# Litianyu141/Pytorch-Sparse-Linalg-torch-amgx.cg.bicg.gmres

Measured on AMD Instinct MI355X. Metric: cg_iters_per_sec, higher is better.
Workload: dtype f64

## Files before the change

pytorch-sparse-linalg-torch-amgx.cg.bicg.gmres_amd/csrc/hipk_cg.hip:

```cpp
#include <type_traits>
#include <math.h>
#include <stdlib.h>

#include <vector>

#include "hipk_blas1.h"
#include "hipk_solve.h"
#include "hipk_spmv.h"
#include "hipk_handoff.h"
#include "hipk_fx.h"

struct hipk_lds_ctl {
    double rs_last;
    int64_t it_done;
    int32_t redo;
    int32_t bar;
    unsigned xcc_mask;
    unsigned pad;
};
struct hipk_cg_scal {
    double gamma[2];
    double atol2;
    double bs;
    double res2;
// ... 949 lines not shown
    }
    if (wg == 0 && tid == 0) {
        a.gamma[it & 1] = gamma;
        scal->rs_last = rs_last;
        scal->it_done = it;
        if (done && it < stop0) *a.stop_it = it;
    }
}

__global__ __launch_bounds__(HIPK_THREADS) void hipk_cg_final_kernel(hipk_cg_scal *__restrict__ scal, int g,
                                                                     const double *__restrict__ part_res,
                                                                     const double *__restrict__ part_xx) {
    __shared__ double sbuf[2 * HIPK_THREADS];
    double res2, xx;
    hipk_reduce_parts2(part_res, part_xx, g, res2, xx, sbuf);
    if (threadIdx.x == 0) {
        scal->res2 = res2;
        scal->xx = xx;
    }
}


static constexpr int kCg2MaxChunks = 150;

static inline bool hipk_cg_streams_by_size(size_t n, size_t sv) { return 4 * n * sv > (size_t)384 << 20; }

#define HIPK_MID_ROW(W, NCH, PRE)                                                                                          \
    {W, NCH, PRE, hipk_cg_mid_kernel<T, W, NCH, PRE>,                                                                      \
     HIPK_FORM_OF_T(T, "hipk_cg_mid_kernel<", #W "," #NCH "," #PRE ">")}
template <typename T>
static const hipk_mid_entry<hipk_cg_mid_args> hipk_cg_mid_table[] = {
    HIPK_MID_ROW(5, 1, false), HIPK_MID_ROW(7, 1, false), HIPK_MID_ROW(9, 1, false), HIPK_MID_ROW(12, 1, false),
    HIPK_MID_ROW(5, 2, false), HIPK_MID_ROW(7, 2, false),
    HIPK_MID_ROW(5, 1, true),  HIPK_MID_ROW(7, 1, true),  HIPK_MID_ROW(9, 1, true),  HIPK_MID_ROW(12, 1, true)};
#undef HIPK_MID_ROW
static constexpr int kPcgMidMaxChunks = 256;
static constexpr size_t kPcgMidSlotBytes = 3 * (size_t)kMidMaxChunks * 256;

struct hipk_cg_layout {
    size_t scal;
    size_t part_a, part_b, part_c;
    size_t part_z[2];
    size_t part_d;
    size_t r, p, Ap;
    size_t lds_flags;
    size_t lds_rr_sub;
    size_t lds_rz_sub;
    bool mid;
    size_t ll_bytes;
    size_t r_ll;
    size_t pap_ll, rr_ll, rz_ll;
    bool fourth_vector;
    size_t p2;
    size_t fuse_words, fuse_ctl;
    size_t total;
};
static constexpr size_t kFuseBytes = 2 * (kFuseWordsBytes + kFuseCtlBytes);
static_assert(kFuseWordsBytes % 256 == 0 && kFuseCtlBytes == 8 * 16 * kFuseReplicaSlots, "the replicas follow the words, 128 bytes apart");
static_assert(kFuseBytes == 2 * (kFuseWordsBytes + kFuseCtlBytes) && (kFuseWordsBytes + kFuseCtlBytes) % 256 == 0,
              "the direction tail's words and replicas follow the first pair, laid out the same");
static_assert(kFuseBytes <= (size_t)kMidMaxChunks * HIPK_BASE_CHUNK * sizeof(double),
              "the fused form runs beyond the mid loop's chunk count, fp64: Ap is longer than its region");
static constexpr size_t kMidSlotArray = (size_t)kMidMaxChunks * 256;
static_assert(kMidSlotBytes == 2 * kMidSlotArray && kPcgMidSlotBytes == 3 * kMidSlotArray, "pap_ll, rr_ll and (pcg) rz_ll");
static_assert(HIPK_MAX_PARTS / 2 + 2 * kHoMaxWg <= HIPK_MAX_PARTS, "the LDS loop's hand-off flags fit the upper half of the spare slot");
static_assert(kHoMaxWg <= HIPK_MAX_PARTS, "the LDS loop's sub-partials fit a chunk-partial slot");
static_assert(kMidSlotBytes >= 256, "p2 ends inside the mid loop's bytes: 2 vec <= ll_bytes + 256");
static_assert(HIPK_SCRATCH_SLOTS == 4, "cg: part_a, part_b, part_c and one unused slot");

static hipk_cg_layout hipk_cg_make_layout(int64_t n, int dtype, bool pre) {
    const size_t sv = (dtype == HIPK_F64) ? 8 : 4, rows = (size_t)(n > 0 ? n : 1), vec = hipk_align_up(rows * sv, 256);
    const size_t slot = HIPK_MAX_PARTS * sizeof(double);
    const hipk_geom gm = hipk_make_geom(n > 0 ? n : 1);
    hipk_cg_layout L;
    hipk_carve take;
    L.scal = take(256);
    L.part_a = take(slot);
    L.part_b = take(slot);
    L.part_c = take(slot);
    L.part_z[0] = take(slot);
    L.part_z[1] = pre ? take(slot) : 0;
    L.part_d = pre ? take(slot) : L.part_a;
    L.lds_flags = L.part_c + slot / 2;
    L.lds_rr_sub = L.part_b;
    L.lds_rz_sub = L.part_z[1];
    L.r = take(vec);
    L.p = take(vec);
    L.mid = gm.g > kMidMinChunks && gm.g <= (pre ? kPcgMidMaxChunks : kMidMaxChunks);
    L.ll_bytes = hipk_align_up(rows * 16, 256);
    L.Ap = L.r_ll = take(L.mid ? L.ll_bytes : vec);
    L.pap_ll = L.mid ? take(pre ? kPcgMidSlotBytes : kMidSlotBytes) : 0;
    L.rr_ll = L.pap_ll + kMidSlotArray;
    L.rz_ll = L.rr_ll + kMidSlotArray;
    const bool second_p = !pre && !L.mid && gm.g > kMidMaxChunks && !hipk_cg_streams_by_size(rows, sv);
    L.p2 = L.Ap + vec;
    if (second_p) take(vec);
    L.fourth_vector = !pre && (L.mid || second_p);
    L.fuse_words = L.Ap;
    L.fuse_ctl = L.Ap + kFuseWordsBytes;
    L.total = take.o;
    return L;
}
extern "C" size_t hipk_cg_work_bytes(int64_t n, int dtype) { return hipk_cg_make_layout(n, dtype, false).total; }
extern "C" size_t hipk_pcg_work_bytes(int64_t n, int dtype) { return hipk_cg_make_layout(n, dtype, true).total; }

struct hipk_cg_path {
    bool small = false;
    bool streams = false;
    bool flat_dir = false;
    bool mid = false;
    const hipk_mid_entry<hipk_cg_mid_args> *mid_entry = nullptr;
    hipk_mid_plan mid_plan;
    size_t mid_lds = 0;
    int nch = 1, slot_stride = 16, xcd_aware = 1;
    bool lds_loop = false;
    bool spread = false;
    bool local = false;
    int64_t max_its = 0;
    bool two_launch = false;
    bool defer_x = false;
    bool fuse_update = false;
    bool fuse_dir = false;
    bool fuse_keep_p = false;
    void (*fuse_kern)(hipk_spmv_args, hipk_cg_fuse_args) = nullptr;
    hipk_spmv_args fuse_sa;
};

template <typename T, bool PRE>
static hipk_cg_path hipk_cg_path_begin(hipk_csr_s *A, const hipk_params *prm, int64_t maxiter, bool mid_failed, hipStream_t stream) {
    const int64_t n = A->n_rows;
    const int g = A->geom.g;
    hipk_cg_path path;
    if (!PRE) {
        path.small = g <= 8 && !hipk_sw_present("HIPK_CG_NO_SMALL");
        path.streams = hipk_sw_force("HIPK_CG_STREAMS", hipk_cg_streams_by_size((size_t)n, sizeof(T)));
        path.flat_dir = hipk_sw_force("HIPK_CG_FLAT_DIRECTION", (size_t)n * sizeof(T) > ((size_t)256 << 20));
    }
    path.nch = (PRE || g <= A->n_cu) ? 1 : 2;
    const int nch = path.nch;
    path.mid_entry = hipk_mid_pick(hipk_cg_mid_table<T>, A->max_row_len, nch, PRE);
    auto mid_lds = [nch](int slots) { return hipk_cg_mid_lds_bytes(slots * HIPK_TILE, nch, PRE, sizeof(T)); };
    path.mid = g > kMidMinChunks && g <= (PRE ? kPcgMidMaxChunks : kMidMaxChunks) && (!PRE || g <= A->n_cu) && A->geom.ch == HIPK_BASE_CHUNK &&
               A->op_cb == nullptr && A->crow != nullptr && A->max_row_len <= 12 && prm->profile == 0 && maxiter > 0 && !mid_failed &&
               hipk_sw_enabled("HIPK_CG_MID") && !hipk_sw_present("HIPK_CG_NO_LDS_LOOP") && !hipk_sw_present("HIPK_CG_NO_SMALL") &&
               path.mid_entry && hipk_mid_eligible(A, path.mid_entry, (g + nch - 1) / nch, mid_lds, stream, &path.mid_plan, &path.mid_lds);
    if (path.mid) {
        const int stride = g <= 32 ? 1 : g <= 256 ? 16 : 4;
        path.slot_stride = PRE ? stride : (int)hipk_sw_int("HIPK_CG_MID_STRIDE", stride);
        if (path.slot_stride < 1 || path.slot_stride > 16) path.slot_stride = 16;
        path.xcd_aware = PRE || hipk_sw_enabled("HIPK_CG_MID_XCD");
        path.max_its = hipk_sw_int("HIPK_CG_LAUNCH_ITS", 16384, 1);
    }
// ... 641 lines not shown
        const int grid1 = ((ntiles + 7) >> 3) << 3;
        for (; it <= maxiter; ++it) {
            HIPK_CHECK_HIP(pace.gate(it, stream, &stop));
            if (stop <= it) break;
            ca.it = it;
            ca.p_old = pbuf[it & 1];
            ca.p_new = pbuf[(it + 1) & 1];
            hipk_cg2_spmv_kernel<T, kCap2><<<grid1, HIPK_THREADS, 0, stream>>>(ca);
            if (it < maxiter)
                hipk_cg2_update_kernel<T><<<gm.g, HIPK_THREADS, 0, stream>>>(n, gm.ch, gm.g, scal, it, A->tile_part, ntiles, Ap,
                                                                            (const T *)pbuf[(it + 1) & 1], r, x, part_b);
            if ((it & 63) == 63) HIPK_CHECK_HIP(hipGetLastError());
        }
        if (it > maxiter) it = maxiter;
        return HIPK_OK;
    }

    int deferred_x_sequence() {
        T *pbuf[2] = {p_first ? hipk_at<T>(work, lay.p2) : p, p_first ? p : hipk_at<T>(work, lay.p2)};
        const int64_t it0 = it;
        if (path.fuse_update) HIPK_TRY(fuse_begin());
        for (; it < maxiter; ++it) {
            HIPK_CHECK_HIP(pace.gate(it, stream, &stop));
            if (stop <= it) break;
            const int j = (int)((it - it0) & 1);
            if (path.fuse_dir) {
                fuse_launch(it0, pbuf[j], pbuf[j ^ 1], j ? x : nullptr);
                if ((it & 63) == 63) HIPK_CHECK_HIP(hipGetLastError());
                continue;
            }
            if (path.fuse_update) {
                fuse_launch(it0, pbuf[j]);
            } else {
                sa.it = it;
                sa.x = sa.w = pbuf[j];
                HIPK_TRY(hipk_launch_spmv(A, sa, stream, &prof));
                hipk_cg_update_kernel<T><<<gm.g, HIPK_THREADS, 0, stream>>>(n, gm.ch, gm.g, scal, it, part_a, Ap, r, part_b, 0, &scal->alpha[it & 1]);
            }
            if (j == 0)
                hipk_cg_pdir_kernel<T><<<gm.g, HIPK_THREADS, 0, stream>>>(n, gm.ch, gm.g, scal, it, maxiter, part_b, r, pbuf[0], pbuf[1]);
            else
                hipk_cg_xdir_kernel<T><<<gm.g, HIPK_THREADS, 0, stream>>>(n, gm.ch, gm.g, scal, it, maxiter, part_b, r, pbuf[1], pbuf[0], x);
            if ((it & 63) == 63) HIPK_CHECK_HIP(hipGetLastError());
        }
        hipk_cg_xflush_kernel<T><<<gm.g, HIPK_THREADS, 0, stream>>>(n, gm.ch, scal, it, it0, pbuf[0], x, path.fuse_dir ? 1 : 0);
        return path.fuse_update ? fuse_end(it0, true, pbuf) : HIPK_OK;
    }

    int fuse_begin() {
        HIPK_CHECK_HIP(hipMemsetAsync(hipk_at<char>(work, lay.fuse_words), 0, kFuseBytes, stream));
        HIPK_CHECK_HIP(hipMemsetAsync(&scal->ctl, 0, sizeof(hipk_lds_ctl), stream));
        fuse_give_up_at = hipk_sw_present("HIPK_TEST_CG_FUSE_GIVE_UP") ? hipk_sw_int("HIPK_TEST_CG_FUSE_GIVE_UP", -1) : -1;
        fuse_dir_give_up_at = hipk_sw_present("HIPK_TEST_CG_FUSE_DIR_GIVE_UP") ? hipk_sw_int("HIPK_TEST_CG_FUSE_DIR_GIVE_UP", -1) : -1;
        fuse_note();
        return HIPK_OK;
    }
    void fuse_note() const {
        char name[64];
        snprintf(name, sizeof(name), "hipk_cg_fuse_update_kernel<%d>", A->sell_w);
        hipk_note_spmv_kernel(name);
    }
    void fuse_launch(int64_t it0, const T *pk, T *p_next = nullptr, T *xq = nullptr) {
        hipk_spmv_args fa = path.fuse_sa;
        fa.it = it;
        fa.x = fa.w = pk;
        hipk_cg_fuse_args ff;
        ff.scal = (hipk_cg_scal *)scal;
        ff.r = (double *)r;
        ff.part_rr = part_b;
        ff.part_pap = part_a;
        ff.words = hipk_at<char>(work, lay.fuse_words);
        ff.ctl = hipk_at<char>(work, lay.fuse_ctl);
        ff.seq = (unsigned)(it - it0) + 1u;
        ff.give_up = it == fuse_give_up_at ? 1 : 0;
        ff.p_next = (double *)p_next;
        ff.x = (double *)xq;
        ff.maxiter = maxiter;
        ff.keep_p = p_next != nullptr && path.fuse_keep_p ? 1 : 0;
        ff.dir_give_up = p_next != nullptr && it == fuse_dir_give_up_at ? 1 : 0;
        path.fuse_kern<<<hipk_xcd_grid(gm.g), HIPK_THREADS, 0, stream>>>(fa, ff);
    }
    int fuse_end(int64_t it0, bool deferred, T *const *pbuf = nullptr) {
        S hs;
        HIPK_CHECK_HIP(hipGetLastError());
        HIPK_CHECK_HIP(hipMemcpyAsync(&hs, scal, sizeof(hs), hipMemcpyDeviceToHost, stream));
        HIPK_CHECK_HIP(hipStreamSynchronize(stream));
        const int64_t ran = (hs.stop_it < it ? hs.stop_it : it) - it0;
        if (path.fuse_dir) hipk_cg_fused_directions += ran > 0 ? ran : 0;
        if (path.fuse_keep_p) hipk_cg_fused_kept_p += ran > 0 ? ran : 0;
        if (hs.ctl.redo == -3) {
            hipk_set_error("hipk_cg_solve: the collector of the fused SpMV + update launch stopped arriving");
            return HIPK_ERR_HIP;
        }
        const bool dir_gave_up = path.fuse_dir && hs.ctl.redo == kFuseDirGaveUp;
        if (hs.ctl.redo != -1 && !dir_gave_up) return HIPK_OK;
        A->cg_fuse_failed = 1;
        path.fuse_update = path.fuse_dir = path.fuse_keep_p = false;
        it = hs.stop_it;
        stop = INT64_MAX;
        HIPK_CHECK_HIP(hipMemcpyAsync(&scal->stop_it, &stop, sizeof(int64_t), hipMemcpyHostToDevice, stream));
        HIPK_CHECK_HIP(hipMemsetAsync(&scal->ctl, 0, sizeof(hipk_lds_ctl), stream));
        HIPK_CHECK_HIP(hipStreamSynchronize(stream));
        HIPK_CHECK_HIP(pace.resume(it));
        if (dir_gave_up) {
            const int j = (int)((it - it0) & 1);
            hipk_cg_pdir_kernel<T><<<gm.g, HIPK_THREADS, 0, stream>>>(n, gm.ch, gm.g, scal, it, maxiter, part_b, r, pbuf[j], pbuf[j ^ 1]);
            if (j == 0) hipk_cg_xflush_kernel<T><<<gm.g, HIPK_THREADS, 0, stream>>>(n, gm.ch, scal, it + 1, it, pbuf[0], x);
            HIPK_CHECK_HIP(hipGetLastError());
            ++it;
        }
        if (deferred) p_first ^= (int)((it - it0) & 1);
        return HIPK_HANDED_BACK;
    }
    int64_t fuse_give_up_at = -1, fuse_dir_give_up_at = -1;

    hipk_cg_kernels<T> pick() const {
        if (path.small)
            return {hipk_cg_update_kernel<T, true>, hipk_cg_direction_kernel<T, true>, A->tile_part, ntiles, HIPK_FORM("cg three-launch, small")};
        if (path.streams && path.flat_dir)
            return {hipk_cg_update_kernel<T, false, true>, nullptr, part_a, 0, HIPK_FORM("cg three-launch, streams + flat direction")};
        if (path.streams)
            return {hipk_cg_update_kernel<T, false, true>, hipk_cg_direction_kernel<T, false, true>, part_a, 0, HIPK_FORM("cg three-launch, streams")};
        return {hipk_cg_update_kernel<T>, hipk_cg_direction_kernel<T>, part_a, 0, HIPK_FORM("cg three-launch")};
    }

    int three_launch_sequence(const hipk_cg_kernels<T> &k) {
        const int64_t it0 = it;
        if (path.fuse_update) HIPK_TRY(fuse_begin());
        for (; it < maxiter; ++it) {
            HIPK_CHECK_HIP(pace.gate(it, stream, &stop));
            if (stop <= it) break;
            if (path.fuse_update) {
                fuse_launch(it0, p);
            } else {
                sa.it = it;
                HIPK_TRY(hipk_launch_spmv(A, sa, stream, &prof));
                hipk_launch_timed(&prof, HIPK_K_UPDATE, k.update, gm.g, HIPK_THREADS, 0, stream, n, gm.ch, gm.g, scal, it, k.pap, Ap, r, part_b, k.ntiles,
                                  (double *)nullptr);
            }
            if (k.direction) {
                hipk_launch_timed(&prof, HIPK_K_DIRECTION, k.direction, gm.g, HIPK_THREADS, 0, stream, n, gm.ch, gm.g, scal, it, maxiter, k.pap, part_b, r,
                                  p, x, k.ntiles);
            } else {
                hipk_launch_timed(&prof, HIPK_K_SCALARS, hipk_cg_scalars_kernel, 1, HIPK_THREADS, 0, stream, gm.g, scal, it, maxiter, part_a, part_b);
                hipk_launch_timed(&prof, HIPK_K_DIRECTION, hipk_cg_direction_flat_kernel<T>, (unsigned)((n + HIPK_BASE_CHUNK - 1) / HIPK_BASE_CHUNK),
                                  HIPK_THREADS, 0, stream, n, scal, it, r, p, x);
            }
            if ((it & 63) == 63) HIPK_CHECK_HIP(hipGetLastError());
        }
        return path.fuse_update ? fuse_end(it0, false) : HIPK_OK;
    }

    int jacobi_sequence() {
        for (; it < maxiter; ++it) {
            HIPK_CHECK_HIP(pace.gate(it, stream, &stop));
            if (stop <= it) break;
            sa.it = it;
            HIPK_TRY(hipk_launch_spmv(A, sa, stream));
            hipk_pcg_update_kernel<T><<<gm.g, HIPK_THREADS, 0, stream>>>(n, gm.ch, gm.g, scal, it, part_a, part_z[it & 1], Ap, dinv, r, part_b,
                                                                          part_z[(it + 1) & 1]);
            hipk_pcg_direction_kernel<T><<<gm.g, HIPK_THREADS, 0, stream>>>(n, gm.ch, gm.g, scal, it, maxiter, part_a, part_z[it & 1],
                                                                             part_z[(it + 1) & 1], part_b, r, dinv, p, x);
            if ((it & 63) == 63) HIPK_CHECK_HIP(hipGetLastError());
        }
        return HIPK_OK;
    }

// ... 210 lines not shown
```

pytorch-sparse-linalg-torch-amgx.cg.bicg.gmres_amd/csrc/hipk_cg_fuse.h:

```cpp
#pragma once
#include "hipk_coded.h"
#include "hipk_mid.h"

static constexpr unsigned kFuseGaveUp = 0x80000000u;
static constexpr unsigned kFuseReplicaSlots = 8;
static constexpr size_t kFuseCtlBytes = 8 * 128;
static constexpr size_t kFuseWordsBytes = (size_t)HIPK_MAX_PARTS * 16;
static constexpr int kFuseDirGaveUp = -4;
static constexpr unsigned kFuseWaitBound = 1u << 24;

struct hipk_cg_fuse_args {
    hipk_cg_scal *scal;
    double *r;
    double *part_rr;
    double *part_pap;
    void *words;
    void *ctl;
    unsigned seq;
    int give_up;
    double *p_next;
    double *x;
    int64_t maxiter;
    int keep_p;
    int dir_give_up;
};

template <int UNITS>
__global__ __launch_bounds__(HIPK_THREADS) HIPK_SGPR80 void hipk_cg_fuse_update_kernel(hipk_spmv_args a, hipk_cg_fuse_args f) {
    typedef double T;
    constexpr int VEC = hipk_vec<T>::VEC, N0 = HIPK_BASE_CHUNK / (VEC * HIPK_THREADS);
    constexpr unsigned STEP = VEC * HIPK_THREADS;
    static_assert(HIPK_MAX_PARTS / HIPK_THREADS == 8, "the collector's poll: eight words per thread");
    static_assert(N0 == HIPK_FUSE_TPC / 2 && VEC == 2, "step k of the tail is the walk's tile 2 k + (wave >> 1), two rows per lane");
    __shared__ double s_pap;
    __shared__ int s_fail;
    hipk_wide_chunk wc;
    T pv[N0][VEC];
    if (!hipk_sell_wide_walk<UNITS, HIPK_SPMV_DOT_W, 0, true>(a, &wc, pv)) return;
    const int t = threadIdx.x, lane = t & 63;
    const int wave = __builtin_amdgcn_readfirstlane(t >> 6);
    const int c = wc.chunk;
    const int64_t base = (int64_t)c * HIPK_BASE_CHUNK;
    const int lim = (int)((base + HIPK_BASE_CHUNK < a.n) ? HIPK_BASE_CHUNK : a.n - base);
    T *const rb = f.r + base;
    const unsigned o0 = VEC * t;
    const double gamma = f.scal->gamma[a.it & 1];
    if (t == 0) s_fail = 0;
    __syncthreads();

    T rv[N0][VEC];
    auto request_r = [&]() {
#pragma unroll
        for (int k = 0; k < N0; ++k) {
            const int o = (int)(o0 + k * STEP);
            const int nv = (lim - o < VEC) ? lim - o : VEC;
            if (nv > 0) hipk_ld<T>((const T *)rb, o, nv, rv[k]);
        }
    };
    if (blockIdx.x != 0) request_r();
    const hipk_ll_rsrc ws = hipk_ll_make(f.words, (size_t)a.g * 16), cs = hipk_ll_make(f.ctl, kFuseCtlBytes);
    if (wave == 0) {
        const double part = hipk_wave_fold(wc.wsum0, wc.cnt, lane);
        if (lane == 0) {
            hipk_ll_put(ws, (unsigned)c, part, f.seq);
            f.part_pap[c] = part;
        }
    }
    if (blockIdx.x == 0) {
#pragma unroll
        for (int k = 0; k < N0; ++k) pv[k][0] = pv[k][1] = (T)0;
        double acc = 0.0;
        if (f.give_up) {
            if (t == 0) s_fail = 1;
        } else {
            constexpr int NK = HIPK_MAX_PARTS / HIPK_THREADS / 2;
            acc = hipk_mid_poll<NK>(ws, a.g, f.seq, &s_fail, 1);
            acc = hipk_mid_poll<NK>(ws, a.g - NK * HIPK_THREADS, f.seq, &s_fail, 1, NK * HIPK_THREADS * 16, acc);
        }
        request_r();
        const double pap = hipk_block_sum(acc, wc.free256);
        const int failed = s_fail;
        if (t < 8) hipk_ll_put(cs, (unsigned)t * kFuseReplicaSlots, pap, failed ? (f.seq | kFuseGaveUp) : f.seq);
        if (failed) {
            if (t == 0) {
                f.scal->stop_it = a.it;
                f.scal->ctl.redo = -1;
                hipk_signal(f.scal->host_sig, HIPK_SIG_STOP | a.it);
            }
            return;
        }
        if (t == 0) s_pap = pap;
    } else if (t == 0) {
        const unsigned slot = (blockIdx.x & 7) * kFuseReplicaSlots;
        hipk_v4u w = hipk_ll_load(cs, slot);
        unsigned spins = 0;
        int bad = 0;
        while (!(w.y == w.w && (w.y & ~kFuseGaveUp) == f.seq)) {
            __builtin_amdgcn_s_sleep(1);
            if (++spins > kFuseWaitBound) {
                f.scal->ctl.redo = -3;
                f.scal->stop_it = a.it;
                hipk_signal(f.scal->host_sig, HIPK_SIG_STOP | a.it);
                bad = 1;
                break;
            }
            w = hipk_ll_load(cs, slot);
        }
        if (bad || (w.y & kFuseGaveUp)) s_fail = 1;
        s_pap = hipk_ll_val(w);
    }
    __syncthreads();
    if (s_fail) return;
    const T alpha = (T)(gamma / s_pap);
    if (c == 0 && t == 0) f.scal->alpha[a.it & 1] = (double)alpha;
    double acc = 0.0;
#pragma unroll
    for (int k = 0; k < N0; ++k) {
        const int o = (int)(o0 + k * STEP);
        const int nv = (lim - o < VEC) ? lim - o : VEC;
        if (nv > 0) {
            const double2 ap = *(const double2 *)(wc.stage + o);
            const T av[VEC] = {ap.x, ap.y};
            T out[VEC];
#pragma unroll
            for (int e = 0; e < VEC; ++e) {
                const T m1 = alpha * av[e];
                out[e] = rv[k][e] - m1;
                if (e < nv) acc = fma((double)out[e], (double)out[e], acc);
                rv[k][e] = out[e];
            }
            hipk_st<T>(rb, o, nv, out);
        }
    }
    acc = hipk_block_sum(acc, wc.free256);
    if (t == 0) f.part_rr[c] = acc;
    if (f.p_next == nullptr) return;

    char *const region2 = (char *)f.ctl + kFuseCtlBytes;
    const hipk_ll_rsrc ws2 = hipk_ll_make(region2, (size_t)a.g * 16), cs2 = hipk_ll_make(region2 + kFuseWordsBytes, kFuseCtlBytes);
    if (t == 0) hipk_ll_put(ws2, (unsigned)c, acc, f.seq);
    const T *const pb = (const T *)a.x + base;
    T *const qb = f.p_next + base;
    const unsigned kept = (f.keep_p && blockIdx.x != 0) ? wc.kept : 0u;
    auto request_p = [&]() {
#pragma unroll
        for (int k = 0; k < N0; ++k) {
            const int o = (int)(o0 + k * STEP);
            const int nv = (lim - o < VEC) ? lim - o : VEC;
            if (nv > 0 && !((kept >> k) & 1u)) hipk_ld<T>(pb, o, nv, pv[k]);
        }
        if (f.x != nullptr) {
            T *const xb = f.x + base;
            const T alpha_prev = (T)f.scal->alpha[(a.it - 1) & 1];
#pragma unroll
            for (int k = 0; k < N0; ++k) {
                const int o = (int)(o0 + k * STEP);
                const int nv = (lim - o < VEC) ? lim - o : VEC;
                if (nv > 0) {
                    T xv[VEC], qv[VEC];
                    hipk_ld<T>((const T *)xb, o, nv, xv);
                    hipk_ld<T>((const T *)qb, o, nv, qv);
#pragma unroll
                    for (int e = 0; e < VEC; ++e) {
                        const T m0 = alpha_prev * qv[e];
                        const T x1 = xv[e] + m0;
                        const T m1 = alpha * pv[k][e];
                        xv[e] = x1 + m1;
                    }
                    hipk_st<T>(xb, o, nv, xv);
                }
            }
        }
    };
    if (blockIdx.x == 0) {
#pragma unroll
        for (int k = 0; k < N0; ++k) pv[k][0] = pv[k][1] = (T)0;
#pragma unroll
        for (int k = 0; k < N0; ++k) *(double2 *)(wc.stage + o0 + k * STEP) = make_double2(rv[k][0], rv[k][1]);
        asm volatile("" ::: "memory");
        double s = 0.0;
        if (f.dir_give_up) {
            if (t == 0) s_fail = 1;
        } else {
            constexpr int NK = HIPK_MAX_PARTS / HIPK_THREADS / 4;
#pragma unroll
            for (int q = 0; q < 4; ++q) s = hipk_mid_poll<NK>(ws2, a.g - q * NK * HIPK_THREADS, f.seq, &s_fail, 1, q * NK * HIPK_THREADS * 16, s);
        }
        const double rr = hipk_block_sum(s, wc.free256);
        const int failed = s_fail;
        if (t < 8) hipk_ll_put(cs2, (unsigned)t * kFuseReplicaSlots, rr, failed ? (f.seq | kFuseGaveUp) : f.seq);
        if (t == 0) {
            if (failed) {
                f.scal->stop_it = a.it;
                if (__hip_atomic_load(&f.scal->ctl.redo, __ATOMIC_RELAXED, __HIP_MEMORY_SCOPE_AGENT) != -3) f.scal->ctl.redo = kFuseDirGaveUp;
                hipk_signal(f.scal->host_sig, HIPK_SIG_STOP | a.it);
            } else {
                s_pap = rr;
                hipk_cg_dir_done(f.scal, a.it, f.maxiter, rr);
            }
        }
        request_p();
#pragma unroll
        for (int k = 0; k < N0; ++k) {
            const double2 rk = *(const double2 *)(wc.stage + o0 + k * STEP);
            rv[k][0] = rk.x;
            rv[k][1] = rk.y;
        }
    } else {
        request_p();
        if (t == 0) {
            const unsigned slot = (blockIdx.x & 7) * kFuseReplicaSlots;
            hipk_v4u w = hipk_ll_load(cs2, slot);
            unsigned spins = 0;
            int bad = 0;
            while (!(w.y == w.w && (w.y & ~kFuseGaveUp) == f.seq)) {
                __builtin_amdgcn_s_sleep(1);
                if (++spins > kFuseWaitBound) {
                    f.scal->ctl.redo = -3;
                    f.scal->stop_it = a.it;
                    hipk_signal(f.scal->host_sig, HIPK_SIG_STOP | a.it);
                    bad = 1;
                    break;
                }
                w = hipk_ll_load(cs2, slot);
            }
            if (bad || (w.y & kFuseGaveUp)) s_fail = 1;
            s_pap = hipk_ll_val(w);
        }
    }
    __syncthreads();
    if (s_fail) return;
    const T beta = (T)(s_pap / gamma);
#pragma unroll
    for (int k = 0; k < N0; ++k) {
        const int o = (int)(o0 + k * STEP);
        const int nv = (lim - o < VEC) ? lim - o : VEC;
        if (nv > 0) {
            T pn[VEC];
#pragma unroll
            for (int e = 0; e < VEC; ++e) {
                const T m = beta * pv[k][e];
                pn[e] = rv[k][e] + m;
            }
            hipk_st<T>(qb, o, nv, pn);
        }
    }
}
```

pytorch-sparse-linalg-torch-amgx.cg.bicg.gmres_amd/csrc/hipk_switch.h:

```cpp
#pragma once
#include <cstdint>
#include <cstdlib>
#include <cstring>

enum hipk_sw_kind {
    HIPK_SW_PRESENT,
    HIPK_SW_OFF_IF_0,
    HIPK_SW_FORCE01,
    HIPK_SW_INT,
    HIPK_SW_WORD,
};
struct hipk_sw_row {
    const char *name;
    hipk_sw_kind kind;
    const char *dflt, *read, *meaning, *used_by;
};

static constexpr hipk_sw_row hipk_switches[] = {
    {"HIPK_SPMV_CODED", HIPK_SW_OFF_IF_0, "on", "handle creation", "0: build neither coded form, plain CSR kernels only", "test, tools A/B"},
    {"HIPK_SPMV_OFFSET_CODED", HIPK_SW_OFF_IF_0, "on", "handle creation", "0: skip the offset-coded form (variable coefficients stay on the CSR kernels)", "test"},
    {"HIPK_SPMV_CODED_LAYOUT", HIPK_SW_WORD, "sliced-ELL planes", "handle creation", "csr: pair codes in CSR order + row lengths; any other word is the default", "test, tools A/B"},
    {"HIPK_SPMV_UNIFORM", HIPK_SW_OFF_IF_0, "on", "handle creation", "0: no uniform-tile words, the coded SpMV reads every tile's code planes", "test"},
    {"HIPK_SPMV_MASKED", HIPK_SW_FORCE01, "off", "handle creation", "1: build the masked-tile analysis (fp64 pair codes); measured slower", "test"},
    {"HIPK_SPMV_SELL_CHUNKED", HIPK_SW_INT, "2", "handle creation; whether set: first coded SpMV of the process", "k: chunk-per-workgroup form when k x chunks >= resident workgroups; < 0 reads as 0 (never), 1 reads as 2 (quirk, kept); set at all also turns off the factor 4 of the two-rows-per-lane kernel", "test, tools A/B"},
    {"HIPK_SPMV_SELL_LOOP", HIPK_SW_INT, "1", "handle creation", "k: persistent grid = k x the resident workgroups, clamped to 1 .. 4", "test, tools A/B"},
    {"HIPK_SPMV_NO_PLAN_CACHE", HIPK_SW_PRESENT, "off", "first coded SpMV of the process", "resolve the coded SpMV's dispatch per launch instead of once per (handle, mode, geometry)", "test, tools A/B"},
    {"HIPK_SPMV_SELL_NO_MODE", HIPK_SW_PRESENT, "off", "first coded SpMV of the process", "run-time instead of compiled-in mode bits in the pair / two-rows-per-lane kernels", "test, tools A/B"},
    {"HIPK_SPMV_SELL_NO_WIDE", HIPK_SW_PRESENT, "off", "each SpMV dispatch", "the one-row-per-lane coded kernels instead of the two-rows-per-lane kernel", "test, tools A/B"},
    {"HIPK_SPMV_SELL_STRIDED", HIPK_SW_INT, "automatic", "each SpMV dispatch", "0 | nonzero: force the chunk walk | the grouped walk of the coded kernels (unset: by tiles per chunk)", "test, tools A/B"},
    {"HIPK_SPMV_SELL_NO_PAIR", HIPK_SW_PRESENT, "off", "first chunked coded SpMV of the process", "the one-tile-per-trip coded kernel instead of the pair kernel", "test, tools A/B"},
    {"HIPK_CHEB_FUSED", HIPK_SW_OFF_IF_0, "on", "each hipk_cheb_apply", "0: every Chebyshev step as SpMV + hipk_cheb_step_kernel instead of the SpMV's Chebyshev epilogue (same bits)", "test, tools A/B"},
    {"HIPK_HOST_SIGNAL", HIPK_SW_OFF_IF_0, "on", "each solve", "0: follow the loop with stream-ordered reads of the device stop word instead of the pinned-host signal word", "test"},
    {"HIPK_PACE_TIMEOUT_US", HIPK_SW_INT, "200000", "each solve", "t: microseconds the signal word may stand still before the stream-ordered fallback; negative: ignored", "test"},
    {"HIPK_PACE_WINDOW", HIPK_SW_INT, "8", "each solve", "k: iterations the host may run ahead of the GPU; outside 1 .. 4096: ignored", "test, user"},
    {"HIPK_TEST_LDS_NOT_RESIDENT", HIPK_SW_INT, "unset", "each one-launch loop; each hand-back", "k: the k-th launch of a one-launch loop reports its workgroups as not co-resident, k < 2 (0 included) reads as 1; set at all: a hand-back does not set the process-wide latch", "test"},
    {"HIPK_NO_LDS_SPREAD", HIPK_SW_PRESENT, "off", "each solve", "9 .. 32 chunks: the launch sequences instead of the one-launch kernels spread over the chip (cg, bicgstab, gmres)", "test, tools A/B"},
    {"HIPK_CG_NO_SMALL", HIPK_SW_PRESENT, "off", "each CG solve", "general launch sequence also for <= 8 reduction chunks; also keeps both one-launch loops away", "test"},
    {"HIPK_CG_NO_LDS_LOOP", HIPK_SW_PRESENT, "off", "each CG solve", "launch sequences instead of either one-launch loop (mid and LDS)", "test, tools A/B"},
    {"HIPK_CG_MID", HIPK_SW_OFF_IF_0, "on", "each CG solve", "0: no hipk_cg_mid_kernel; the LDS loop up to 32 chunks, else the launch sequences", "test, tools A/B"},
    {"HIPK_CG_MID_STRIDE", HIPK_SW_INT, "by chunk count", "each launch of the mid loop, plain CG only", "k: chunk-partial slots k x 16 B apart; outside 1 .. 16 reads as 16", "tools A/B"},
    {"HIPK_CG_MID_XCD", HIPK_SW_OFF_IF_0, "on", "each launch of the mid loop, plain CG only", "0: workgroup b takes row range b (no XCD-aware placement)", "tools A/B"},
    {"HIPK_CG_LAUNCH_ITS", HIPK_SW_INT, "16384", "each one-launch loop", "k: iterations one launch of a one-launch CG loop may run, at least 1", "test"},
    {"HIPK_CG_LOOP_AGENT", HIPK_SW_PRESENT, "off", "each LDS loop", "agent-scope hand-offs in hipk_cg_solve_lds_kernel also on one XCD", "test"},
    {"HIPK_CG_TWO_LAUNCH", HIPK_SW_OFF_IF_0, "on", "each plain CG solve", "0: the three-launch iteration instead of hipk_cg2_spmv_kernel + hipk_cg2_update_kernel", "test, tools A/B"},
    {"HIPK_CG_DEFER_X", HIPK_SW_OFF_IF_0, "on", "each plain CG solve", "0: every direction launch updates x (hipk_cg_direction_kernel)", "test, tools A/B"},
    {"HIPK_CG_FUSE_UPDATE", HIPK_SW_FORCE01, "automatic", "each plain CG solve", "0 | 1: the SpMV and the update step as two launches | as hipk_cg_fuse_update_kernel where the form applies (unset: fused where it applies)", "test, tools A/B"},
    {"HIPK_CG_FUSE_DIRECTION", HIPK_SW_FORCE01, "automatic", "each plain CG solve", "0 | 1: the direction step of the fused deferred-x sequence as hipk_cg_pdir_kernel / hipk_cg_xdir_kernel launches | as the tail of hipk_cg_fuse_update_kernel where the form applies (unset: the tail where it applies)", "test, tools A/B"},
    {"HIPK_CG_FUSE_KEEP_P", HIPK_SW_OFF_IF_0, "on", "each plain CG solve", "0: the direction tail of hipk_cg_fuse_update_kernel loads all of p_k again instead of keeping the uniform tiles' rows in the walk's registers (same bits)", "test, tools A/B"},
    {"HIPK_TEST_CG_FUSE_DIR_GIVE_UP", HIPK_SW_INT, "unset", "each fused CG sequence", "k: the collector of the direction tail's hand-off at iteration k behaves as if its poll had run out (the solve goes on with the separate kernels)", "test"},
    {"HIPK_TEST_CG_FUSE_GIVE_UP", HIPK_SW_INT, "unset", "each fused CG sequence", "k: the collector of hipk_cg_fuse_update_kernel at iteration k behaves as if its poll had run out (the solve goes on with the separate kernels)", "test"},
    {"HIPK_CG_STREAMS", HIPK_SW_FORCE01, "automatic", "each plain CG solve", "0 | 1: force the vector kernels' cache policy (unset: streams when x, r, p, Ap exceed 384 MiB)", "test"},
    {"HIPK_CG_FLAT_DIRECTION", HIPK_SW_FORCE01, "automatic", "each plain CG solve", "0 | 1: with the streaming policy, the direction step per chunk | as scalars launch + flat grid (unset: flat when a vector exceeds 256 MiB)", "test, tools A/B"},
    {"HIPK_BICGSTAB_NO_SMALL", HIPK_SW_PRESENT, "off", "each BiCGStab solve", "general launch sequence also for <= 8 reduction chunks; also keeps both one-launch loops away", "test"},
    {"HIPK_BICGSTAB_NO_LDS_LOOP", HIPK_SW_PRESENT, "off", "each BiCGStab solve", "five launches per iteration instead of either one-launch loop (mid and LDS)", "test, tools A/B"},
    {"HIPK_BICGSTAB_MID", HIPK_SW_OFF_IF_0, "on", "each BiCGStab solve", "0: no hipk_bi_mid_kernel; the LDS loop up to 32 chunks, else the launch sequence", "test, tools A/B"},
    {"HIPK_BICGSTAB_LAUNCH_ITS", HIPK_SW_INT, "8192", "each one-launch loop", "k: iterations one launch of a one-launch BiCGStab loop may run, at least 1", "test"},
    {"HIPK_BICGSTAB_LOOP_AGENT", HIPK_SW_PRESENT, "off", "each LDS loop", "agent-scope hand-offs in hipk_bi_solve_lds_kernel also on one XCD", "test"},
    {"HIPK_GMRES_NO_SMALL", HIPK_SW_PRESENT, "off", "each GMRES solve", "general launch sequence also for <= 8 reduction chunks; also keeps the spread whole-solve kernel away", "test"},
    {"HIPK_GMRES_NO_WIDE", HIPK_SW_PRESENT, "off", "each GMRES solve", "small systems: the 256-thread multi-dot / update kernels instead of the wide ones (and no one-launch cycle)", "test"},
    {"HIPK_GMRES_NO_CYCLE", HIPK_SW_PRESENT, "off", "each GMRES solve", "one launch per kernel instead of any one-launch cycle (small, LDS, mid)", "test, tools A/B"},
    {"HIPK_GMRES_NO_LDS_CYCLE", HIPK_SW_PRESENT, "off", "each GMRES solve", "hipk_gm_cycle_small_kernel (one launch per restart cycle) instead of hipk_gm_solve_lds_kernel", "test, tools A/B"},
    {"HIPK_GM_CYCLE_AGENT", HIPK_SW_PRESENT, "off", "each GMRES solve", "agent-scope hand-offs in hipk_gm_solve_lds_kernel also on one XCD", "test"},
    {"HIPK_GM_LAUNCH_CYCLES", HIPK_SW_INT, "64", "each launch of a one-launch cycle", "k: restart cycles one launch of hipk_gm_solve_lds_kernel may run (no clamp)", "test"},
    {"HIPK_GMRES_NO_STREAM", HIPK_SW_PRESENT, "off", "each GMRES solve", "large systems, restart <= 31: the first multi-dot / update kernels instead of the streaming ones", "test, tools A/B"},
    {"HIPK_GMRES_MID", HIPK_SW_OFF_IF_0, "on", "each GMRES solve", "0: the launch sequence per Arnoldi step instead of hipk_gm_mid_kernel", "test, tools A/B"},
    {"HIPK_GMRES_MID_MIN", HIPK_SW_INT, "32", "each GMRES solve", "k: hipk_gm_mid_kernel from k + 1 chunks, floor 8 (A/B against the whole-solve kernel of 9 .. 32 chunks)", "tools A/B"},
    {"HIPK_GM_MD_WIDE", HIPK_SW_INT, "0", "each GMRES solve", "nonzero: multi-dot with up to 32 columns per workgroup; measured slower", "tools A/B"},
    {"HIPK_GM_SPLIT_NORM", HIPK_SW_INT, "by chunk count", "each GMRES solve", "0 | nonzero: the one-kernel normalise step | scalars launch + flat scale kernel (large systems)", "test, tools A/B"},
    {"HIPK_GM_NRES", HIPK_SW_INT, "5", "each GMRES solve", "k: basis columns read with the default cache policy, the rest non-temporal (no clamp)", "test, tools A/B"},
    {"HIPK_GM_SPEC", HIPK_SW_INT, "1", "each GMRES solve", "second CGS pass launched at every step (0), where predicted (1), or learned from scratch (2)", "test, tools A/B"},
    {"HIPK_GM_STAMPS", HIPK_SW_PRESENT, "off", "each launch and the end of a small-system GMRES solve", "stamps build only: print the per-phase shader clocks of the cycle kernels", "tools A/B"},
    {"HIPK_BATCH_LAUNCH_ITS", HIPK_SW_INT, "16384", "each batch solve", "k: iterations per system one launch of a batch kernel may run, at least 1", "test"},
    {"HIPK_DIST_OVERLAP", HIPK_SW_INT, "0", "each hipk_dist_cg_solve", "nonzero: x += alpha p on a side stream beside the second collective; measured slower", "test"},
    {"HIPK_DIST_FUSED", HIPK_SW_OFF_IF_0, "on", "each hipk_dist_cg_solve", "0: the collective entry points also on a communicator with a fused area", "user"},
};

constexpr bool hipk_sw_streq(const char *a, const char *b) {
    while (*a && *a == *b) ++a, ++b;
    return *a == *b;
}
constexpr bool hipk_sw_is_row(const char *name, hipk_sw_kind kind, bool any = false) {
    for (const hipk_sw_row &r : hipk_switches)
        if (hipk_sw_streq(r.name, name)) return any || r.kind == kind;
    return false;
}
template <bool in_table>
struct hipk_sw_checked {
    static_assert(in_table, "not a row of hipk_switches, or a row of another kind");
    static const char *get(const char *name) { return getenv(name); }
};
#define HIPK_SW_GET(name, ...) (hipk_sw_checked<hipk_sw_is_row(name, __VA_ARGS__)>::get(name))

#define hipk_sw_present(name) (HIPK_SW_GET(name, HIPK_SW_PRESENT, true) != nullptr)
#define hipk_sw_enabled(name) hipk_sw_parse_enabled(HIPK_SW_GET(name, HIPK_SW_OFF_IF_0))
#define hipk_sw_force(name, automatic) hipk_sw_parse_force(HIPK_SW_GET(name, HIPK_SW_FORCE01), (automatic))
#define hipk_sw_int(name, ...) hipk_sw_parse_int(HIPK_SW_GET(name, HIPK_SW_INT), __VA_ARGS__)
#define hipk_sw_word_is(name, word) hipk_sw_parse_word(HIPK_SW_GET(name, HIPK_SW_WORD), (word))

static inline bool hipk_sw_parse_enabled(const char *e) { return !(e && e[0] == '0'); }
static inline bool hipk_sw_parse_force(const char *e, bool automatic) { return e ? e[0] == '1' : automatic; }
static inline int64_t hipk_sw_parse_int(const char *e, int64_t dflt, int64_t lo = INT64_MIN, int64_t hi = INT64_MAX) {
    const int64_t v = e ? (int64_t)atoll(e) : dflt;
    return v < lo ? lo : v > hi ? hi : v;
// ... 3 lines not shown
```

Before: 23600.

## Split fused CG reduction collector into eight parallel collectors with replicated hand-out

```diff
diff --git a/pytorch-sparse-linalg-torch-amgx.cg.bicg.gmres_amd/csrc/hipk_cg.hip b/pytorch-sparse-linalg-torch-amgx.cg.bicg.gmres_amd/csrc/hipk_cg.hip
--- a/pytorch-sparse-linalg-torch-amgx.cg.bicg.gmres_amd/csrc/hipk_cg.hip
+++ b/pytorch-sparse-linalg-torch-amgx.cg.bicg.gmres_amd/csrc/hipk_cg.hip
@@ -1025,7 +1025,7 @@
     size_t pap_ll, rr_ll, rz_ll;
     bool fourth_vector;
     size_t p2;
-    size_t fuse_words, fuse_ctl;
+    size_t fuse_words;
     size_t total;
 };
 static constexpr size_t kFuseBytes = 2 * (kFuseWordsBytes + kFuseCtlBytes);
@@ -1070,7 +1070,6 @@
     if (second_p) take(vec);
     L.fourth_vector = !pre && (L.mid || second_p);
     L.fuse_words = L.Ap;
-    L.fuse_ctl = L.Ap + kFuseWordsBytes;
     L.total = take.o;
     return L;
 }
@@ -1818,6 +1817,8 @@
         HIPK_CHECK_HIP(hipMemsetAsync(&scal->ctl, 0, sizeof(hipk_lds_ctl), stream));
         fuse_give_up_at = hipk_sw_present("HIPK_TEST_CG_FUSE_GIVE_UP") ? hipk_sw_int("HIPK_TEST_CG_FUSE_GIVE_UP", -1) : -1;
         fuse_dir_give_up_at = hipk_sw_present("HIPK_TEST_CG_FUSE_DIR_GIVE_UP") ? hipk_sw_int("HIPK_TEST_CG_FUSE_DIR_GIVE_UP", -1) : -1;
+        const int64_t who = hipk_sw_present("HIPK_TEST_CG_FUSE_GIVE_UP_WHO") ? hipk_sw_int("HIPK_TEST_CG_FUSE_GIVE_UP_WHO", -1) : -1;
+        fuse_give_up_who = who >= 0 && who < (int64_t)kFuseCollectors ? 1 << (int)who : (1 << kFuseCollectors) - 1;
         fuse_note();
         return HIPK_OK;
     }
@@ -1836,14 +1837,12 @@
         ff.part_rr = part_b;
         ff.part_pap = part_a;
         ff.words = hipk_at<char>(work, lay.fuse_words);
-        ff.ctl = hipk_at<char>(work, lay.fuse_ctl);
         ff.seq = (unsigned)(it - it0) + 1u;
-        ff.give_up = it == fuse_give_up_at ? 1 : 0;
+        ff.give_up = (it == fuse_give_up_at ? fuse_give_up_who : 0) | (p_next != nullptr && it == fuse_dir_give_up_at ? fuse_give_up_who << 8 : 0);
         ff.p_next = (double *)p_next;
         ff.x = (double *)xq;
         ff.maxiter = maxiter;
         ff.keep_p = p_next != nullptr && path.fuse_keep_p ? 1 : 0;
-        ff.dir_give_up = p_next != nullptr && it == fuse_dir_give_up_at ? 1 : 0;
         path.fuse_kern<<<hipk_xcd_grid(gm.g), HIPK_THREADS, 0, stream>>>(fa, ff);
     }
     int fuse_end(int64_t it0, bool deferred, T *const *pbuf = nullptr) {
@@ -1855,7 +1854,7 @@
         if (path.fuse_dir) hipk_cg_fused_directions += ran > 0 ? ran : 0;
         if (path.fuse_keep_p) hipk_cg_fused_kept_p += ran > 0 ? ran : 0;
         if (hs.ctl.redo == -3) {
-            hipk_set_error("hipk_cg_solve: the collector of the fused SpMV + update launch stopped arriving");
+            hipk_set_error("hipk_cg_solve: a collector of the fused SpMV + update launch stopped arriving");
             return HIPK_ERR_HIP;
         }
         const bool dir_gave_up = path.fuse_dir && hs.ctl.redo == kFuseDirGaveUp;
@@ -1879,6 +1878,7 @@
         return HIPK_HANDED_BACK;
     }
     int64_t fuse_give_up_at = -1, fuse_dir_give_up_at = -1;
+    int fuse_give_up_who = (1 << kFuseCollectors) - 1;
 
     hipk_cg_kernels<T> pick() const {
         if (path.small)
diff --git a/pytorch-sparse-linalg-torch-amgx.cg.bicg.gmres_amd/csrc/hipk_cg_fuse.h b/pytorch-sparse-linalg-torch-amgx.cg.bicg.gmres_amd/csrc/hipk_cg_fuse.h
--- a/pytorch-sparse-linalg-torch-amgx.cg.bicg.gmres_amd/csrc/hipk_cg_fuse.h
+++ b/pytorch-sparse-linalg-torch-amgx.cg.bicg.gmres_amd/csrc/hipk_cg_fuse.h
@@ -3,10 +3,12 @@
 #include "hipk_mid.h"
 
 static constexpr unsigned kFuseGaveUp = 0x80000000u;
+static constexpr unsigned kFuseCollectors = 8;
 static constexpr unsigned kFuseReplicaSlots = 8;
 static constexpr size_t kFuseCtlBytes = 8 * 128;
 static constexpr size_t kFuseWordsBytes = (size_t)HIPK_MAX_PARTS * 16;
 static constexpr int kFuseDirGaveUp = -4;
+__host__ __device__ constexpr unsigned hipk_fuse_word_slot(unsigned c) { return (c % kFuseCollectors) * HIPK_THREADS + c / kFuseCollectors; }
 static constexpr unsigned kFuseWaitBound = 1u << 24;
 
 struct hipk_cg_fuse_args {
@@ -15,22 +17,79 @@
     double *part_rr;
     double *part_pap;
     void *words;
-    void *ctl;
     unsigned seq;
     int give_up;
     double *p_next;
     double *x;
     int64_t maxiter;
     int keep_p;
-    int dir_give_up;
 };
+
+__device__ __forceinline__ double hipk_fuse_class_sum(hipk_ll_rsrc ws, int g, unsigned seq, int s, int skip, int *fail, double *sb) {
+    const int u = threadIdx.x, j = u & 31;
+    const int mine = s + 8 * j + (u >> 5) * 256;
+    if (skip) {
+        if (u == 0) *fail = 1;
+    } else if (mine < g) {
+        double v = 0.0;
+        const unsigned slot = hipk_fuse_word_slot((unsigned)mine);
+        if (!hipk_ll_wait(ws, slot, seq, hipk_ll_load(ws, slot), v)) *fail = 1;
+        sb[u] = v;
+    }
+    __syncthreads();
+    double acc = 0.0;
+    if (u < 64) {
+        if (!skip) {
+#pragma unroll
+            for (int i = 0; i < HIPK_MAX_PARTS / HIPK_THREADS; ++i)
+                if (s + 8 * j + i * 256 < g) acc = acc + sb[32 * i + j];
+        }
+        acc = hipk_half_sum(acc);
+    }
+    return acc;
+}
+__device__ __forceinline__ void hipk_fuse_hand_out(hipk_ll_rsrc cs, int s, double sum, unsigned seq, int failed, int lane) {
+    const double v = __hiloint2double(__builtin_amdgcn_readfirstlane(__double2hiint(sum)), __builtin_amdgcn_readfirstlane(__double2loint(sum)));
+    if (lane < (int)kFuseCollectors) hipk_ll_put(cs, (unsigned)lane * kFuseReplicaSlots + (unsigned)s, v, failed ? (seq | kFuseGaveUp) : seq);
+}
+__device__ __forceinline__ double hipk_fuse_wait(hipk_ll_rsrc cs, unsigned line, unsigned seq, hipk_cg_scal *scal, int64_t it, int lane, int *fail) {
+    const unsigned slot = line * kFuseReplicaSlots + (unsigned)(lane & 7);
+    hipk_v4u w = {0u, 0u, 0u, 0u};
+    unsigned spins = 0;
+    int bad = 0;
+    for (;;) {
+        if (lane < (int)kFuseCollectors) w = hipk_ll_load(cs, slot);
+        const bool whole = lane < (int)kFuseCollectors && w.y == w.w && (w.y & ~kFuseGaveUp) == seq;
+        if (__ballot(whole && (w.y & kFuseGaveUp)) != 0ull) {
+            bad = 1;
+            break;
+        }
+        if ((__ballot(whole) & 0xFFull) == 0xFFull) break;
+        __builtin_amdgcn_s_sleep(1);
+        if (++spins > kFuseWaitBound) {
+            if (lane == 0) {
+                scal->ctl.redo = -3;
+                scal->stop_it = it;
+                hipk_signal(scal->host_sig, HIPK_SIG_STOP | it);
+            }
+            bad = 1;
+            break;
+        }
+    }
+    if (bad && lane == 0) *fail = 1;
+    double v = hipk_ll_val(w);
+    v = v + hipk_row_shl<4>(v);
+    v = v + hipk_row_shl<2>(v);
+    v = v + hipk_row_shl<1>(v);
+    return v;
+}
 
 template <int UNITS>
 __global__ __launch_bounds__(HIPK_THREADS) HIPK_SGPR80 void hipk_cg_fuse_update_kernel(hipk_spmv_args a, hipk_cg_fuse_args f) {
     typedef double T;
     constexpr int VEC = hipk_vec<T>::VEC, N0 = HIPK_BASE_CHUNK / (VEC * HIPK_THREADS);
     constexpr unsigned STEP = VEC * HIPK_THREADS;
-    static_assert(HIPK_MAX_PARTS / HIPK_THREADS == 8, "the collector's poll: eight words per thread");
+    static_assert(HIPK_MAX_PARTS == kFuseCollectors * HIPK_THREADS, "a collector's poll: one word per thread");
     static_assert(N0 == HIPK_FUSE_TPC / 2 && VEC == 2, "step k of the tail is the walk's tile 2 k + (wave >> 1), two rows per lane");
     __shared__ double s_pap;
     __shared__ int s_fail;
@@ -48,66 +107,39 @@
     if (t == 0) s_fail = 0;
     __syncthreads();
 
+    const bool collector = blockIdx.x < kFuseCollectors;
+    const unsigned line = blockIdx.x & 7;
     T rv[N0][VEC];
-    auto request_r = [&]() {
-#pragma unroll
-        for (int k = 0; k < N0; ++k) {
-            const int o = (int)(o0 + k * STEP);
-            const int nv = (lim - o < VEC) ? lim - o : VEC;
-            if (nv > 0) hipk_ld<T>((const T *)rb, o, nv, rv[k]);
-        }
-    };
-    if (blockIdx.x != 0) request_r();
-    const hipk_ll_rsrc ws = hipk_ll_make(f.words, (size_t)a.g * 16), cs = hipk_ll_make(f.ctl, kFuseCtlBytes);
+#pragma unroll
+    for (int k = 0; k < N0; ++k) {
+        const int o = (int)(o0 + k * STEP);
+        const int nv = (lim - o < VEC) ? lim - o : VEC;
+        if (nv > 0) hipk_ld<T>((const T *)rb, o, nv, rv[k]);
+    }
+    const hipk_ll_rsrc ws = hipk_ll_make(f.words, kFuseWordsBytes), cs = hipk_ll_make((char *)f.words + kFuseWordsBytes, kFuseCtlBytes);
     if (wave == 0) {
         const double part = hipk_wave_fold(wc.wsum0, wc.cnt, lane);
         if (lane == 0) {
-            hipk_ll_put(ws, (unsigned)c, part, f.seq);
+            hipk_ll_put(ws, hipk_fuse_word_slot((unsigned)c), part, f.seq);
             f.part_pap[c] = part;
         }
     }
-    if (blockIdx.x == 0) {
-#pragma unroll
-        for (int k = 0; k < N0; ++k) pv[k][0] = pv[k][1] = (T)0;
-        double acc = 0.0;
-        if (f.give_up) {
-            if (t == 0) s_fail = 1;
-        } else {
-            constexpr int NK = HIPK_MAX_PARTS / HIPK_THREADS / 2;
-            acc = hipk_mid_poll<NK>(ws, a.g, f.seq, &s_fail, 1);
-            acc = hipk_mid_poll<NK>(ws, a.g - NK * HIPK_THREADS, f.seq, &s_fail, 1, NK * HIPK_THREADS * 16, acc);
-        }
-        request_r();
-        const double pap = hipk_block_sum(acc, wc.free256);
-        const int failed = s_fail;
-        if (t < 8) hipk_ll_put(cs, (unsigned)t * kFuseReplicaSlots, pap, failed ? (f.seq | kFuseGaveUp) : f.seq);
-        if (failed) {
-            if (t == 0) {
+    if (collector) {
+        const int cls = (int)blockIdx.x;
+        const double sum = hipk_fuse_class_sum(ws, a.g, f.seq, cls, (f.give_up >> cls) & 1, &s_fail, wc.free256);
+        if (wave == 0) {
+            const int failed = s_fail;
+            hipk_fuse_hand_out(cs, cls, sum, f.seq, failed, t);
+            if (failed && t == 0) {
                 f.scal->stop_it = a.it;
                 f.scal->ctl.redo = -1;
                 hipk_signal(f.scal->host_sig, HIPK_SIG_STOP | a.it);
             }
-            return;
-        }
+        }
+    }
+    if (wave == 0) {
+        const double pap = hipk_fuse_wait(cs, line, f.seq, f.scal, a.it, t, &s_fail);
         if (t == 0) s_pap = pap;
-    } else if (t == 0) {
-        const unsigned slot = (blockIdx.x & 7) * kFuseReplicaSlots;
-        hipk_v4u w = hipk_ll_load(cs, slot);
-        unsigned spins = 0;
-        int bad = 0;
-        while (!(w.y == w.w && (w.y & ~kFuseGaveUp) == f.seq)) {
-            __builtin_amdgcn_s_sleep(1);
-            if (++spins > kFuseWaitBound) {
-                f.scal->ctl.redo = -3;
-                f.scal->stop_it = a.it;
-                hipk_signal(f.scal->host_sig, HIPK_SIG_STOP | a.it);
-                bad = 1;
-                break;
-            }
-            w = hipk_ll_load(cs, slot);
-        }
-        if (bad || (w.y & kFuseGaveUp)) s_fail = 1;
-        s_pap = hipk_ll_val(w);
     }
     __syncthreads();
     if (s_fail) return;
@@ -136,96 +168,58 @@
     if (t == 0) f.part_rr[c] = acc;
     if (f.p_next == nullptr) return;
 
-    char *const region2 = (char *)f.ctl + kFuseCtlBytes;
-    const hipk_ll_rsrc ws2 = hipk_ll_make(region2, (size_t)a.g * 16), cs2 = hipk_ll_make(region2 + kFuseWordsBytes, kFuseCtlBytes);
-    if (t == 0) hipk_ll_put(ws2, (unsigned)c, acc, f.seq);
+    char *const region2 = (char *)f.words + kFuseWordsBytes + kFuseCtlBytes;
+    const hipk_ll_rsrc ws2 = hipk_ll_make(region2, kFuseWordsBytes), cs2 = hipk_ll_make(region2 + kFuseWordsBytes, kFuseCtlBytes);
+    if (t == 0) hipk_ll_put(ws2, hipk_fuse_word_slot((unsigned)c), acc, f.seq);
+    if (collector) {
+        const int cls = (int)blockIdx.x;
+        const double sum = hipk_fuse_class_sum(ws2, a.g, f.seq, cls, (f.give_up >> (8 + cls)) & 1, &s_fail, wc.free256);
+        if (wave == 0) {
+            const int failed = s_fail;
+            hipk_fuse_hand_out(cs2, cls, sum, f.seq, failed, t);
+            if (failed && t == 0) {
+                f.scal->stop_it = a.it;
+                if (__hip_atomic_load(&f.scal->ctl.redo, __ATOMIC_RELAXED, __HIP_MEMORY_SCOPE_AGENT) != -3) f.scal->ctl.redo = kFuseDirGaveUp;
+                hipk_signal(f.scal->host_sig, HIPK_SIG_STOP | a.it);
+            }
+        }
+    }
     const T *const pb = (const T *)a.x + base;
     T *const qb = f.p_next + base;
-    const unsigned kept = (f.keep_p && blockIdx.x != 0) ? wc.kept : 0u;
-    auto request_p = [&]() {
+    const unsigned kept = f.keep_p ? wc.kept : 0u;
+#pragma unroll
+    for (int k = 0; k < N0; ++k) {
+        const int o = (int)(o0 + k * STEP);
+        const int nv = (lim - o < VEC) ? lim - o : VEC;
+        if (nv > 0 && !((kept >> k) & 1u)) hipk_ld<T>(pb, o, nv, pv[k]);
+    }
+    if (f.x != nullptr) {
+        T *const xb = f.x + base;
+        const T alpha_prev = (T)f.scal->alpha[(a.it - 1) & 1];
 #pragma unroll
         for (int k = 0; k < N0; ++k) {
             const int o = (int)(o0 + k * STEP);
             const int nv = (lim - o < VEC) ? lim - o : VEC;
-            if (nv > 0 && !((kept >> k) & 1u)) hipk_ld<T>(pb, o, nv, pv[k]);
-        }
-        if (f.x != nullptr) {
-            T *const xb = f.x + base;
-            const T alpha_prev = (T)f.scal->alpha[(a.it - 1) & 1];
-#pragma unroll
-            for (int k = 0; k < N0; ++k) {
-                const int o = (int)(o0 + k * STEP);
-                const int nv = (lim - o < VEC) ? lim - o : VEC;
-                if (nv > 0) {
-                    T xv[VEC], qv[VEC];
-                    hipk_ld<T>((const T *)xb, o, nv, xv);
-                    hipk_ld<T>((const T *)qb, o, nv, qv);
-#pragma unroll
-                    for (int e = 0; e < VEC; ++e) {
-                        const T m0 = alpha_prev * qv[e];
-                        const T x1 = xv[e] + m0;
-                        const T m1 = alpha * pv[k][e];
-                        xv[e] = x1 + m1;
-                    }
-                    hipk_st<T>(xb, o, nv, xv);
+            if (nv > 0) {
+                T xv[VEC], qv[VEC];
+                hipk_ld<T>((const T *)xb, o, nv, xv);
+                hipk_ld<T>((const T *)qb, o, nv, qv);
+#pragma unroll
+                for (int e = 0; e < VEC; ++e) {
+                    const T m0 = alpha_prev * qv[e];
+                    const T x1 = xv[e] + m0;
+                    const T m1 = alpha * pv[k][e];
+                    xv[e] = x1 + m1;
                 }
-            }
-        }
-    };
-    if (blockIdx.x == 0) {
-#pragma unroll
-        for (int k = 0; k < N0; ++k) pv[k][0] = pv[k][1] = (T)0;
-#pragma unroll
-        for (int k = 0; k < N0; ++k) *(double2 *)(wc.stage + o0 + k * STEP) = make_double2(rv[k][0], rv[k][1]);
-        asm volatile("" ::: "memory");
-        double s = 0.0;
-        if (f.dir_give_up) {
-            if (t == 0) s_fail = 1;
-        } else {
-            constexpr int NK = HIPK_MAX_PARTS / HIPK_THREADS / 4;
-#pragma unroll
-            for (int q = 0; q < 4; ++q) s = hipk_mid_poll<NK>(ws2, a.g - q * NK * HIPK_THREADS, f.seq, &s_fail, 1, q * NK * HIPK_THREADS * 16, s);
-        }
-        const double rr = hipk_block_sum(s, wc.free256);
-        const int failed = s_fail;
-        if (t < 8) hipk_ll_put(cs2, (unsigned)t * kFuseReplicaSlots, rr, failed ? (f.seq | kFuseGaveUp) : f.seq);
+                hipk_st<T>(xb, o, nv, xv);
+            }
+        }
+    }
+    if (wave == 0) {
+        const double rr = hipk_fuse_wait(cs2, line, f.seq, f.scal, a.it, t, &s_fail);
         if (t == 0) {
-            if (failed) {
-                f.scal->stop_it = a.it;
-                if (__hip_atomic_load(&f.scal->ctl.redo, __ATOMIC_RELAXED, __HIP_MEMORY_SCOPE_AGENT) != -3) f.scal->ctl.redo = kFuseDirGaveUp;
-                hipk_signal(f.scal->host_sig, HIPK_SIG_STOP | a.it);
-            } else {
-                s_pap = rr;
-                hipk_cg_dir_done(f.scal, a.it, f.maxiter, rr);
-            }
-        }
-        request_p();
-#pragma unroll
-        for (int k = 0; k < N0; ++k) {
-            const double2 rk = *(const double2 *)(wc.stage + o0 + k * STEP);
-            rv[k][0] = rk.x;
-            rv[k][1] = rk.y;
-        }
-    } else {
-        request_p();
-        if (t == 0) {
-            const unsigned slot = (blockIdx.x & 7) * kFuseReplicaSlots;
-            hipk_v4u w = hipk_ll_load(cs2, slot);
-            unsigned spins = 0;
-            int bad = 0;
-            while (!(w.y == w.w && (w.y & ~kFuseGaveUp) == f.seq)) {
-                __builtin_amdgcn_s_sleep(1);
-                if (++spins > kFuseWaitBound) {
-                    f.scal->ctl.redo = -3;
-                    f.scal->stop_it = a.it;
-                    hipk_signal(f.scal->host_sig, HIPK_SIG_STOP | a.it);
-                    bad = 1;
-                    break;
-                }
-                w = hipk_ll_load(cs2, slot);
-            }
-            if (bad || (w.y & kFuseGaveUp)) s_fail = 1;
-            s_pap = hipk_ll_val(w);
+            s_pap = rr;
+            if (blockIdx.x == 0 && !s_fail) hipk_cg_dir_done(f.scal, a.it, f.maxiter, rr);
         }
     }
     __syncthreads();
diff --git a/pytorch-sparse-linalg-torch-amgx.cg.bicg.gmres_amd/csrc/hipk_switch.h b/pytorch-sparse-linalg-torch-amgx.cg.bicg.gmres_amd/csrc/hipk_switch.h
--- a/pytorch-sparse-linalg-torch-amgx.cg.bicg.gmres_amd/csrc/hipk_switch.h
+++ b/pytorch-sparse-linalg-torch-amgx.cg.bicg.gmres_amd/csrc/hipk_switch.h
@@ -47,8 +47,9 @@
     {"HIPK_CG_FUSE_UPDATE", HIPK_SW_FORCE01, "automatic", "each plain CG solve", "0 | 1: the SpMV and the update step as two launches | as hipk_cg_fuse_update_kernel where the form applies (unset: fused where it applies)", "test, tools A/B"},
     {"HIPK_CG_FUSE_DIRECTION", HIPK_SW_FORCE01, "automatic", "each plain CG solve", "0 | 1: the direction step of the fused deferred-x sequence as hipk_cg_pdir_kernel / hipk_cg_xdir_kernel launches | as the tail of hipk_cg_fuse_update_kernel where the form applies (unset: the tail where it applies)", "test, tools A/B"},
     {"HIPK_CG_FUSE_KEEP_P", HIPK_SW_OFF_IF_0, "on", "each plain CG solve", "0: the direction tail of hipk_cg_fuse_update_kernel loads all of p_k again instead of keeping the uniform tiles' rows in the walk's registers (same bits)", "test, tools A/B"},
-    {"HIPK_TEST_CG_FUSE_DIR_GIVE_UP", HIPK_SW_INT, "unset", "each fused CG sequence", "k: the collector of the direction tail's hand-off at iteration k behaves as if its poll had run out (the solve goes on with the separate kernels)", "test"},
-    {"HIPK_TEST_CG_FUSE_GIVE_UP", HIPK_SW_INT, "unset", "each fused CG sequence", "k: the collector of hipk_cg_fuse_update_kernel at iteration k behaves as if its poll had run out (the solve goes on with the separate kernels)", "test"},
+    {"HIPK_TEST_CG_FUSE_DIR_GIVE_UP", HIPK_SW_INT, "unset", "each fused CG sequence", "k: the collectors of the direction tail's hand-off at iteration k behave as if their poll had run out (the solve goes on with the separate kernels)", "test"},
+    {"HIPK_TEST_CG_FUSE_GIVE_UP", HIPK_SW_INT, "unset", "each fused CG sequence", "k: the collectors of hipk_cg_fuse_update_kernel at iteration k behave as if their poll had run out (the solve goes on with the separate kernels)", "test"},
+    {"HIPK_TEST_CG_FUSE_GIVE_UP_WHO", HIPK_SW_INT, "unset", "each fused CG sequence", "s: only collector s (0 .. 7) obeys HIPK_TEST_CG_FUSE_GIVE_UP / HIPK_TEST_CG_FUSE_DIR_GIVE_UP; outside 0 .. 7: ignored (all eight do)", "test"},
     {"HIPK_CG_STREAMS", HIPK_SW_FORCE01, "automatic", "each plain CG solve", "0 | 1: force the vector kernels' cache policy (unset: streams when x, r, p, Ap exceed 384 MiB)", "test"},
     {"HIPK_CG_FLAT_DIRECTION", HIPK_SW_FORCE01, "automatic", "each plain CG solve", "0 | 1: with the streaming policy, the direction step per chunk | as scalars launch + flat grid (unset: flat when a vector exceeds 256 MiB)", "test, tools A/B"},
     {"HIPK_BICGSTAB_NO_SMALL", HIPK_SW_PRESENT, "off", "each BiCGStab solve", "general launch sequence also for <= 8 reduction chunks; also keeps both one-launch loops away", "test"},
```

After: 25070 (median of 6 runs). 6.2% higher.
